# crstnbr/detqmc

Measured on AMD Instinct MI355X. Metric: DQMC sweeps/sec (SDW-O2 L=16 beta=10 fp64), higher is better.
Workload: dtype f64; 1 GPU; DetSDW O(2) L=16 beta=10 dtau=0.1 s=10 checkerboard delayed(32) sweepThermalization, 512 independent chains per GPU (1 process x 4 kernel contexts x 128 lockstep chains), stabilisation=qr; n_g=512, m=100, replicas_per_gpu=512, processes_per_gpu=1, contexts_per_process=4, chains_per_context=128, launch=self

## Files before the change

detqmc_amd/csrc/kernels_bmult.hip:

```cpp
#include "dqmc_internal.h"
#include <algorithm>
#include <cstdlib>
#include <mutex>

__device__ __forceinline__ cplx cadd(cplx a, cplx b) { return make_double2(a.x + b.x, a.y + b.y); }
__device__ __forceinline__ cplx cmul(cplx a, cplx b) {
    return make_double2(a.x * b.x - a.y * b.y, a.x * b.y + a.y * b.x);
}
__device__ __forceinline__ cplx cfma(cplx a, cplx b, cplx c) {
    c.x = fma(a.x, b.x, c.x); c.x = fma(-a.y, b.y, c.x);
    c.y = fma(a.x, b.y, c.y); c.y = fma(a.y, b.x, c.y);
    return c;
}
__device__ __forceinline__ cplx cscale(cplx a, double s) { return make_double2(a.x * s, a.y * s); }

template<int MSF>
__device__ __forceinline__ void build_V(cplx (&V)[MSF][MSF], double sign, double c0, double c1, double xs,
                                        double p0, double p1, double p2) {
#pragma unroll
    for (int a = 0; a < MSF; ++a)
#pragma unroll
        for (int b = 0; b < MSF; ++b) V[a][b] = make_double2(0.0, 0.0);
    cplx bx = make_double2(sign * p0 * xs, -sign * p1 * xs);
    cplx bcx = make_double2(sign * p0 * xs, sign * p1 * xs);
    V[0][0] = make_double2(c0, 0.0);
    V[1][1] = make_double2(c1, 0.0);
    V[0][1] = bx;
    V[1][0] = bcx;
    if (MSF == 4) {
        double ax = sign * p2 * xs;
        V[2][2] = make_double2(c0, 0.0);
        V[3][3] = make_double2(c1, 0.0);
        V[0][3] = make_double2(ax, 0.0);
        V[3][0] = make_double2(ax, 0.0);
        V[1][2] = make_double2(-ax, 0.0);
        V[2][1] = make_double2(-ax, 0.0);
        V[3][2] = bx;
        V[2][3] = bcx;
    }
}

template<int MSF, bool RIGHT, bool INV, bool CDW>
__global__ __launch_bounds__(512, MSF == 2 ? 4 : 2) void k_bmult_chain(DevModel dm, cplx* __restrict__ A, int lda, int nvec,
                                                      int kfirst, int kstep, int kcount, int shift, size_t cs) {
    extern __shared__ cplx sm[];
    dm = chain_model(dm, cs); CHAIN(A);
    const int N = dm.N, ng = dm.ng, P = dm.P;
    const int v0 = blockIdx.x * nvec;
    const int nv = min(nvec, ng - v0);
    if (nv <= 0) return;
    const int tid = threadIdx.x, nth = blockDim.x;
    const int rstride = nvec + 1;
    auto addr = [&](int v, int e) -> int { return RIGHT ? (e * rstride + v) : (v * ng + e); };

    const int rv0 = tid % nvec, re0 = tid / nvec, rvd = nth % nvec, red = nth / nvec;
    constexpr int SB = 8;
    if (!RIGHT) {
        const int total = nv * ng;
        const cplx* src = A + (size_t)v0 * lda;
        for (int base = tid; base < total; base += SB * nth) {
            cplx r[SB];
#pragma unroll
            for (int u = 0; u < SB; ++u) {
                const int idx = min(base + u * nth, total - 1);
                size_t off = idx;
                if (lda != ng) { const int v = idx / ng; off = (size_t)v * lda + (idx - v * ng); }
                r[u] = nt_load(src + off);
            }
#pragma unroll
            for (int u = 0; u < SB; ++u) { const int idx = base + u * nth; if (idx < total) sm[idx] = r[u]; }
        }
    } else {
        int v = rv0, e = re0;
        const int total = nvec * ng;
        for (int base = tid; base < total; base += SB * nth) {
            cplx r[SB];
            int la[SB];
#pragma unroll
            for (int u = 0; u < SB; ++u) {
                la[u] = (base + u * nth < total && v < nv) ? e * rstride + v : -1;
                r[u] = nt_load(A + (size_t)min(e, ng - 1) * lda + (v0 + min(v, nv - 1)));
                v += rvd; e += red;
                if (v >= nvec) { v -= nvec; e += 1; }
            }
#pragma unroll
            for (int u = 0; u < SB; ++u) if (la[u] >= 0) sm[la[u]] = r[u];
        }
    }
    __syncthreads();

    constexpr bool PASSES_FIRST = (RIGHT == INV);
    const int signIdx = INV ? 1 : 0;
    const double vsign = INV ? +1.0 : -1.0;

    int pl0[3], pld[3];
    if (!RIGHT) { pl0[0] = tid % P; pl0[1] = tid / P; pl0[2] = 0; pld[0] = nth % P; pld[1] = nth / P; pld[2] = 0; }
    else {
        pl0[0] = tid % nv; const int t0 = tid / nv; pl0[1] = t0 % P; pl0[2] = t0 / P;
        pld[0] = nth % nv; const int t1 = nth / nv; pld[1] = t1 % P; pld[2] = t1 / P;
    }
    const int si0 = tid % N, sv0 = tid / N, sid = nth % N, svd = nth / N;

    for (int kc = 0; kc < kcount; ++kc) {
        const int k = kfirst + kc * kstep;
        for (int stage = 0; stage < 2; ++stage) {
            const bool do_passes = (stage == 0) == PASSES_FIRST;
            if (shift && !do_passes) continue;
            if (do_passes) {
                if (dm.dense) continue;
                const double* abcd_tab = shift ? dm.pabcd_h : dm.pabcd;
                const cplx* mat_tab = shift ? dm.pmats_h : dm.pmats;
                const int npass = shift ? 2 : 3;
                for (int pass = 0; pass < npass; ++pass) {
                    const int sub = shift ? (pass == 0 ? 1 : 0) : ((pass == 1) ? 0 : 1);
                    if (!shift && pass == (PASSES_FIRST ? npass - 1 : 0)) {
                        const int fitems = nv * P;
                        const double* ph = dm.phi + (size_t)k * dm.opdim * N;
                        for (int idx = tid; idx < fitems; idx += nth) {
                            int p, v;
                            if (RIGHT) { v = idx % nv; p = idx / nv; } else { p = idx % P; v = idx / P; }
                            int site[4];
#pragma unroll
                            for (int q = 0; q < 4; ++q) site[q] = dm.psites[(sub * 4 + q) * P + p];
                            cplx x[MSF][4];
#pragma unroll
                            for (int b = 0; b < MSF; ++b)
#pragma unroll
                                for (int q = 0; q < 4; ++q) x[b][q] = sm[addr(v, b * N + site[q])];
                            auto vmix = [&]() {
#pragma unroll
                                for (int q = 0; q < 4; ++q) {
                                    const int i = site[q];
                                    const double c = dm.coshT[(size_t)k * N + i];
                                    double xs = dm.sinhT[(size_t)k * N + i], c0, c1;
                                    if constexpr (CDW) cdw_site_terms(dm, (size_t)k * N + i, vsign, c, c0, c1, xs); else { c0 = c; c1 = c; }
                                    const double p0 = ph[i];
                                    const double p1 = dm.opdim > 1 ? ph[N + i] : 0.0;
                                    const double p2 = dm.opdim > 2 ? ph[2 * N + i] : 0.0;
                                    cplx V[MSF][MSF];
                                    build_V<MSF>(V, vsign, c0, c1, xs, p0, p1, p2);
                                    cplx in[MSF], out[MSF];
#pragma unroll
                                    for (int b = 0; b < MSF; ++b) in[b] = x[b][q];
                                    if (PASSES_FIRST) {
#pragma unroll
                                        for (int b = 0; b < MSF; ++b) in[b] = cscale(in[b], INV ? dm.ovinv[b & 1] : dm.ov[b & 1]);
                                    }
#pragma unroll
                                    for (int o = 0; o < MSF; ++o) {
                                        cplx acc = make_double2(0.0, 0.0);
#pragma unroll
                                        for (int b = 0; b < MSF; ++b) {
                                            const cplx vv = RIGHT ? V[b][o] : V[o][b];
                                            acc = cfma(vv, in[b], acc);
                                        }
                                        if (!PASSES_FIRST) acc = cscale(acc, INV ? dm.ovinv[o & 1] : dm.ov[o & 1]);
                                        out[o] = acc;
                                    }
#pragma unroll
                                    for (int b = 0; b < MSF; ++b) x[b][q] = out[b];
                                }
                            };
                            if (!PASSES_FIRST) vmix();
#pragma unroll
                            for (int b = 0; b < MSF; ++b) {
                                const int tbl = ((b & 1) * 2 + signIdx) * 2 + sub;
                                cplx y[4];
                                if (dm.pm_real) {
                                    double co[4];
#pragma unroll
                                    for (int q = 0; q < 4; ++q) co[q] = abcd_tab[(tbl * 4 + q) * P + p];
#pragma unroll
                                    for (int a = 0; a < 4; ++a) {
                                        cplx acc = make_double2(0.0, 0.0);
#pragma unroll
                                        for (int q = 0; q < 4; ++q) {
                                            const double m = co[a ^ q];
                                            acc.x = fma(m, x[b][q].x, acc.x);
                                            acc.y = fma(m, x[b][q].y, acc.y);
                                        }
                                        y[a] = acc;
                                    }
                                } else {
                                    const cplx* mat = mat_tab + (size_t)tbl * 16 * P + p;
#pragma unroll
                                    for (int a = 0; a < 4; ++a) {
                                        cplx acc = make_double2(0.0, 0.0);
#pragma unroll
                                        for (int q = 0; q < 4; ++q) {
                                            const cplx mm = RIGHT ? mat[(size_t)(q * 4 + a) * P] : mat[(size_t)(a * 4 + q) * P];
                                            acc = cfma(mm, x[b][q], acc);
                                        }
                                        y[a] = acc;
                                    }
                                }
#pragma unroll
                                for (int q = 0; q < 4; ++q) x[b][q] = y[q];
                            }
                            if (PASSES_FIRST) vmix();
#pragma unroll
                            for (int b = 0; b < MSF; ++b)
#pragma unroll
                                for (int q = 0; q < 4; ++q) sm[addr(v, b * N + site[q])] = x[b][q];
                        }
                        __syncthreads();
                        continue;
                    }
                    const int items = nv * MSF * P;
                    int d0 = pl0[0], d1 = pl0[1], d2 = pl0[2];
                    for (int idx = tid; idx < items; idx += nth) {
                        int p, b, v;
                        if (RIGHT) { v = d0; p = d1; b = d2; }
                        else { p = d0; b = d1 % MSF; v = d1 / MSF; }
                        d0 += pld[0]; d1 += pld[1]; d2 += pld[2];
                        if (RIGHT) { if (d0 >= nv) { d0 -= nv; d1 += 1; } if (d1 >= P) { d1 -= P; d2 += 1; } }
                        else { if (d0 >= P) { d0 -= P; d1 += 1; } }
                        int band = b & 1;
                        const int tbl = (band * 2 + signIdx) * 2 + sub;
                        int e[4];
                        cplx x[4], y[4];
#pragma unroll
                        for (int q = 0; q < 4; ++q) { e[q] = addr(v, b * N + dm.psites[(sub * 4 + q) * P + p]); x[q] = sm[e[q]]; }
                        if (dm.pm_real) {
                            double co[4];
#pragma unroll
                            for (int q = 0; q < 4; ++q) co[q] = abcd_tab[(tbl * 4 + q) * P + p];
#pragma unroll
                            for (int a = 0; a < 4; ++a) {
                                cplx acc = make_double2(0.0, 0.0);
#pragma unroll
                                for (int q = 0; q < 4; ++q) {
                                    const double m = co[a ^ q];
                                    acc.x = fma(m, x[q].x, acc.x);
                                    acc.y = fma(m, x[q].y, acc.y);
                                }
                                y[a] = acc;
                            }
                        } else {
                            const cplx* mat = mat_tab + (size_t)tbl * 16 * P + p;
#pragma unroll
                            for (int a = 0; a < 4; ++a) {
                                cplx acc = make_double2(0.0, 0.0);
#pragma unroll
                                for (int q = 0; q < 4; ++q) {
                                    cplx mm = RIGHT ? mat[(size_t)(q * 4 + a) * P] : mat[(size_t)(a * 4 + q) * P];
                                    acc = cfma(mm, x[q], acc);
                                }
                                y[a] = acc;
                            }
                        }
#pragma unroll
                        for (int q = 0; q < 4; ++q) sm[e[q]] = y[q];
                    }
                    __syncthreads();
                }
            } else {
                if (!dm.dense) continue;
                const int items = nv * N;
                const double* ph = dm.phi + (size_t)k * dm.opdim * N;
                int i = si0, v = sv0, inext, vnext;
                for (int idx = tid; idx < items; idx += nth, i = inext, v = vnext) {
                    inext = i + sid; vnext = v + svd;
                    if (inext >= N) { inext -= N; vnext += 1; }
                    double c = dm.coshT[(size_t)k * N + i], xs = dm.sinhT[(size_t)k * N + i], c0, c1;
                    if constexpr (CDW) cdw_site_terms(dm, (size_t)k * N + i, vsign, c, c0, c1, xs); else { c0 = c; c1 = c; }
                    double p0 = ph[i];
                    double p1 = dm.opdim > 1 ? ph[N + i] : 0.0;
                    double p2 = dm.opdim > 2 ? ph[2 * N + i] : 0.0;
                    cplx V[MSF][MSF];
                    build_V<MSF>(V, vsign, c0, c1, xs, p0, p1, p2);
                    cplx in[MSF], out[MSF];
#pragma unroll
                    for (int q = 0; q < MSF; ++q) in[q] = sm[addr(v, q * N + i)];
                    if (PASSES_FIRST) {
#pragma unroll
                        for (int q = 0; q < MSF; ++q) in[q] = cscale(in[q], INV ? dm.ovinv[q & 1] : dm.ov[q & 1]);
                    }
#pragma unroll
                    for (int o = 0; o < MSF; ++o) {
                        cplx acc = make_double2(0.0, 0.0);
#pragma unroll
                        for (int q = 0; q < MSF; ++q) {
                            cplx vv = RIGHT ? V[q][o] : V[o][q];
                            acc = cfma(vv, in[q], acc);
                        }
                        if (!PASSES_FIRST) acc = cscale(acc, INV ? dm.ovinv[o & 1] : dm.ov[o & 1]);
                        out[o] = acc;
                    }
#pragma unroll
                    for (int q = 0; q < MSF; ++q) sm[addr(v, q * N + i)] = out[q];
                }
                __syncthreads();
            }
        }
    }

    if (!RIGHT) {
        cplx* dst = A + (size_t)v0 * lda;
        for (int idx = tid; idx < nv * ng; idx += nth) {
            size_t off = idx;
            if (lda != ng) { const int v = idx / ng; off = (size_t)v * lda + (idx - v * ng); }
            nt_store(dst + off, sm[idx]);
        }
    } else {
        int v = rv0, e = re0;
        for (int idx = tid; idx < nvec * ng; idx += nth) {
            if (v < nv) nt_store(A + (size_t)e * lda + (v0 + v), sm[e * rstride + v]);
            v += rvd; e += red;
            if (v >= nvec) { v -= nvec; e += 1; }
        }
    }
}

void launch_bmult(const Launch& lc, const DevModel* , const DevModel& hm, int side, int inverse,
                  int kfirst, int kstep, int kcount, cplx* A, int lda, int shift) {
    const int ng = hm.ng;
    const size_t lds_cap = side == DQMC_LEFT ? 65536 : 144 * 1024;
    const int max_fit = (int)(lds_cap / ((size_t)ng * sizeof(cplx))) - (side == DQMC_LEFT ? 0 : 1);
    static const int env_l = dev_knob("DQMC_BMULT_NVEC_L") ? atoi(dev_knob("DQMC_BMULT_NVEC_L")) : 0;
    static const int env_r = dev_knob("DQMC_BMULT_NVEC_R") ? atoi(dev_knob("DQMC_BMULT_NVEC_R")) : 0;
    int nvec;
    if (side == DQMC_LEFT) {
        const int per_pass = (256 + hm.P - 1) / hm.P;
        nvec = env_l ? env_l : std::max(ng / 256, per_pass);
        if (nvec > ng) nvec = ng;
    } else {
        nvec = env_r ? env_r : 8;
    }
    if (nvec > max_fit) nvec = max_fit;
    if (nvec < 1) nvec = 1;
    const int grid = (ng + nvec - 1) / nvec;
    const size_t lds = (size_t)(side == DQMC_LEFT ? nvec : nvec + 1) * ng * sizeof(cplx);
    if (lds > 48 * 1024) {
        static std::mutex mu;
        static size_t raised_tab[64][16] = {};
        int dev = 0;
        (void)hipGetDevice(&dev);
        const int slot = (hm.cdw_on ? 8 : 0) + (hm.MSF == 4 ? 4 : 0) + (side == DQMC_LEFT ? 0 : 2) + (inverse ? 1 : 0);
        std::lock_guard<std::mutex> lk(mu);
        size_t& raised = raised_tab[dev & 63][slot];
        if (lds > raised) {
            const void* f = nullptr;
#define BM_F(MSFV, R, I) (hm.cdw_on ? (const void*)k_bmult_chain<MSFV, R, I, true> : (const void*)k_bmult_chain<MSFV, R, I, false>)
            if (hm.MSF == 2) f = side == DQMC_LEFT ? (inverse ? BM_F(2, false, true) : BM_F(2, false, false)) : (inverse ? BM_F(2, true, true) : BM_F(2, true, false));
            else             f = side == DQMC_LEFT ? (inverse ? BM_F(4, false, true) : BM_F(4, false, false)) : (inverse ? BM_F(4, true, true) : BM_F(4, true, false));
#undef BM_F
            if (hipFuncSetAttribute(f, hipFuncAttributeMaxDynamicSharedMemorySize, (int)lds) == hipSuccess) raised = lds;
            else (void)hipGetLastError();
        }
    }
    static const int env_t = dev_knob("DQMC_BMULT_THREADS_R") ? atoi(dev_knob("DQMC_BMULT_THREADS_R")) : 0;
    const int nthreads = (side == DQMC_LEFT) ? 256 : (env_t ? env_t : (nvec >= 8 ? 512 : 256));
#define LAUNCH(MSFV, R, I)                                                                              \
    do { if (hm.cdw_on) hipLaunchKernelGGL((k_bmult_chain<MSFV, R, I, true>), dim3(grid, 1, lc.nb), dim3(nthreads), lds, lc.st, hm, A, lda, nvec, \
                                           kfirst, kstep, kcount, shift, lc.cs);                        \
         else hipLaunchKernelGGL((k_bmult_chain<MSFV, R, I, false>), dim3(grid, 1, lc.nb), dim3(nthreads), lds, lc.st, hm, A, lda, nvec, \
                                 kfirst, kstep, kcount, shift, lc.cs); } while (0)
    if (hm.MSF == 2) {
        if (side == DQMC_LEFT) { if (!inverse) LAUNCH(2, false, false); else LAUNCH(2, false, true); }
        else                   { if (!inverse) LAUNCH(2, true, false);  else LAUNCH(2, true, true); }
    } else {
        if (side == DQMC_LEFT) { if (!inverse) LAUNCH(4, false, false); else LAUNCH(4, false, true); }
        else                   { if (!inverse) LAUNCH(4, true, false);  else LAUNCH(4, true, true); }
    }
#undef LAUNCH
}

__global__ void k_cosh_sinh(DevModel dm, size_t cs) {
    dm = chain_model(dm, cs);
    const int total = dm.m * dm.N;
    for (int idx = blockIdx.x * blockDim.x + threadIdx.x; idx < total; idx += gridDim.x * blockDim.x) {
        int k = 1 + idx / dm.N, i = idx % dm.N;
        double nn = 0.0;
        for (int d = 0; d < dm.opdim; ++d) {
            double p = dm.phi[((size_t)k * dm.opdim + d) * dm.N + i];
            nn += p * p;
        }
        double nrm = sqrt(nn);
        double a = dm.lambda * dm.dtau * nrm;
        dm.coshT[(size_t)k * dm.N + i] = cosh(a);
        dm.sinhT[(size_t)k * dm.N + i] = sinh(a) / nrm;
    }
}
void launch_cosh_sinh(const Launch& lc, const DevModel& hm) {
    int total = hm.m * hm.N;
    hipLaunchKernelGGL(k_cosh_sinh, dim3((total + 255) / 256, 1, lc.nb), dim3(256), 0, lc.st, hm, lc.cs);
}

__global__ void k_cdw_terms(DevModel dm, size_t cs) {
    dm = chain_model(dm, cs);
    const int total = dm.m * dm.N;
    for (int idx = blockIdx.x * blockDim.x + threadIdx.x; idx < total; idx += gridDim.x * blockDim.x) {
        const size_t e = (size_t)dm.N + idx;
        const double l = dm.cdwl[e];
        const int a = (fabs(l) > 1.5) ? 1 : 0;
        dm.cdwC[e] = dm.cdw_cosh[a];
        dm.cdwS[e] = (l < 0.0) ? -dm.cdw_sinh[a] : dm.cdw_sinh[a];
    }
}
void launch_cdw_terms(const Launch& lc, const DevModel& hm) {
    if (!hm.cdw_on) return;
    int total = hm.m * hm.N;
    hipLaunchKernelGGL(k_cdw_terms, dim3((total + 255) / 256, 1, lc.nb), dim3(256), 0, lc.st, hm, lc.cs);
}

__global__ void k_set_identity(cplx* A, int n, size_t cs) {
    CHAIN(A);
    size_t total = (size_t)n * n;
    for (size_t idx = blockIdx.x * (size_t)blockDim.x + threadIdx.x; idx < total; idx += (size_t)gridDim.x * blockDim.x) {
        int i = (int)(idx % n), j = (int)(idx / n);
        A[idx] = make_double2(i == j ? 1.0 : 0.0, 0.0);
    }
}
void launch_set_identity(const Launch& lc, cplx* A, int n) {
    const int blocks = (int)std::min<size_t>(1024, ((size_t)n * n + 255) / 256);
    hipLaunchKernelGGL(k_set_identity, dim3(blocks, 1, lc.nb), dim3(256), 0, lc.st, A, n, lc.cs);
}

__global__ void k_conj_transpose(const cplx* __restrict__ A, cplx* __restrict__ B, int n, size_t cs) {
    __shared__ cplx tile[32][33];
    CHAIN(A); CHAIN(B);
    int bx = blockIdx.x * 32, by = blockIdx.y * 32;
    int tx = threadIdx.x & 31, ty = threadIdx.x >> 5;
    for (int r = ty; r < 32; r += 8) {
        int i = bx + tx, j = by + r;
        if (i < n && j < n) tile[r][tx] = A[(size_t)j * n + i];
    }
    __syncthreads();
    for (int r = ty; r < 32; r += 8) {
        int i = by + tx, j = bx + r;
        if (i < n && j < n) {
            cplx t = tile[tx][r];
            B[(size_t)j * n + i] = make_double2(t.x, -t.y);
        }
    }
}
void launch_conj_transpose(const Launch& lc, const cplx* A, cplx* B, int n) {
    dim3 grid((n + 31) / 32, (n + 31) / 32, lc.nb);
    hipLaunchKernelGGL(k_conj_transpose, grid, dim3(256), 0, lc.st, A, B, n, lc.cs);
}

__global__ void k_add_diag(cplx* A, const double* d, int n, size_t cs) {
    CHAIN(A); CHAIN(d);
    int i = blockIdx.x * blockDim.x + threadIdx.x;
    if (i < n) A[(size_t)i * n + i].x += d[i];
}
void launch_add_diag(const Launch& lc, cplx* A, const double* d, int n) {
    hipLaunchKernelGGL(k_add_diag, dim3((n + 255) / 256, 1, lc.nb), dim3(256), 0, lc.st, A, d, n, lc.cs);
}

__global__ void k_copy64(const unsigned long long* __restrict__ src, unsigned long long* __restrict__ dst, size_t words, size_t cs) {
    CHAIN(src); CHAIN(dst);
    for (size_t i = blockIdx.x * (size_t)blockDim.x + threadIdx.x; i < words; i += (size_t)gridDim.x * blockDim.x) dst[i] = src[i];
}
void launch_copy_bytes(const Launch& lc, const void* src, void* dst, size_t bytes) {
    if (lc.nb == 1) { (void)hipMemcpyAsync(dst, src, bytes, hipMemcpyDeviceToDevice, lc.st); return; }
    const size_t words = bytes / 8;
    const int blocks = (int)std::min<size_t>(2048, (words + 255) / 256);
    hipLaunchKernelGGL(k_copy64, dim3(blocks, 1, lc.nb), dim3(256), 0, lc.st, (const unsigned long long*)src,
                       (unsigned long long*)dst, words, lc.cs);
}
void launch_copy(const Launch& lc, const cplx* A, cplx* B, size_t count) {
    launch_copy_bytes(lc, A, B, count * sizeof(cplx));
}

__global__ void k_phi_sq_sum(DevModel dm, double* out, size_t cs) {
    __shared__ double red[256];
    dm = chain_model(dm, cs); CHAIN(out);
    double acc = 0.0;
    size_t total = (size_t)dm.m * dm.opdim * dm.N;
    const double* p = dm.phi + (size_t)dm.opdim * dm.N;
    for (size_t idx = threadIdx.x; idx < total; idx += 256) acc += p[idx] * p[idx];
    red[threadIdx.x] = acc;
    __syncthreads();
    for (int s = 128; s > 0; s >>= 1) {
        if ((int)threadIdx.x < s) red[threadIdx.x] += red[threadIdx.x + s];
        __syncthreads();
    }
    if (threadIdx.x == 0) out[0] = red[0];
}
__global__ void k_phi_action(DevModel dm, const DevUpdateState* __restrict__ us, double* out, size_t cs) {
    __shared__ double red[256];
    dm = chain_model(dm, cs); CHAIN(us); CHAIN(out);
    const int N = dm.N, L = dm.L, m = dm.m, OPD = dm.opdim;
    const double dtau = dm.dtau, r = us->r, u = dm.u, c = dm.c;
    double acc = 0.0;
    for (int idx = threadIdx.x; idx < m * N; idx += 256) {
        const int k = 1 + idx / N, site = idx % N;
        const int kprev = (k > 1) ? k - 1 : m;
        const int x = site % L, y = site / L;
        const int xn = y * L + (x + 1) % L, yn = ((y + 1) % L) * L + x;
        double phisq = 0.0, td2 = 0.0, xd2 = 0.0, yd2 = 0.0;
        for (int d = 0; d < OPD; ++d) {
            const double ph = dm.phi[((size_t)k * OPD + d) * N + site];
            const double td = (ph - dm.phi[((size_t)kprev * OPD + d) * N + site]) / dtau;
            const double xd = ph - dm.phi[((size_t)k * OPD + d) * N + xn];
            const double yd = ph - dm.phi[((size_t)k * OPD + d) * N + yn];
            td2 += td * td; xd2 += xd * xd; yd2 += yd * yd; phisq += ph * ph;
        }
        double a = 0.5 * dtau * r * phisq;
        if (!dm.phi2bosons) a += (dtau / (2.0 * c * c)) * td2 + 0.5 * dtau * xd2 + 0.5 * dtau * yd2 + 0.25 * dtau * u * phisq * phisq;
        acc += a;
    }
    red[threadIdx.x] = acc;
    __syncthreads();
    for (int s = 128; s > 0; s >>= 1) {
        if ((int)threadIdx.x < s) red[threadIdx.x] += red[threadIdx.x + s];
        __syncthreads();
    }
    if (threadIdx.x == 0) out[0] = red[0];
}
void launch_phi_action(const Launch& lc, const DevModel& hm, const DevUpdateState* us, double* out) {
    hipLaunchKernelGGL(k_phi_action, dim3(1, 1, lc.nb), dim3(256), 0, lc.st, hm, us, out, lc.cs);
}
__global__ void k_phi_shift(DevModel dm, const double* __restrict__ shifts, size_t cs) {
    dm = chain_model(dm, cs);
    const double* sh = shifts + (size_t)blockIdx.z * dm.opdim;
    const int total = (dm.m + 1) * dm.opdim * dm.N;
    for (int idx = blockIdx.x * blockDim.x + threadIdx.x; idx < total; idx += gridDim.x * blockDim.x)
        dm.phi[idx] += sh[(idx / dm.N) % dm.opdim];
}
void launch_phi_shift(const Launch& lc, const DevModel& hm, const double* shifts) {
    const int total = (hm.m + 1) * hm.opdim * hm.N;
    hipLaunchKernelGGL(k_phi_shift, dim3((total + 255) / 256, 1, lc.nb), dim3(256), 0, lc.st, hm, shifts, lc.cs);
}
void launch_phi_sq_sum(const Launch& lc, const DevModel& hm, double* out) {
    hipLaunchKernelGGL(k_phi_sq_sum, dim3(1, 1, lc.nb), dim3(256), 0, lc.st, hm, out, lc.cs);
}
__global__ void k_gather_scalars(const double* __restrict__ src, size_t cs, int nb, double factor, double* __restrict__ dst) {
    const int b = blockIdx.x * blockDim.x + threadIdx.x;
    if (b < nb) dst[b] = factor * *(const double*)((const char*)src + (size_t)b * cs);
}
void launch_gather_scalars(const Launch& lc, const double* src, double factor, double* dst) {
    hipLaunchKernelGGL(k_gather_scalars, dim3((lc.nb + 63) / 64), dim3(64), 0, lc.st, src, lc.cs, lc.nb, factor, dst);
}
```

Baseline: 283.8 sweeps/s.

## Fuse checkerboard passes across time slices and stream edges from global memory

Restructures the chained B-matrix multiply so the outer sub-lattice pass of one time slice is merged with the matching pass of the next slice, with the potential mixing step folded in. This removes one pass and one barrier per interior slice. Optionally the first pass reads directly from global memory and the last pass writes directly back, skipping the bulk shared-memory load and store. Defaults enable all three for right multiplies and only the mid fusion for left; this relies on the pass-1 sub-lattice operators composing, and the direct global accesses are scattered rather than coalesced.

```diff
diff --git a/detqmc_amd/csrc/kernels_bmult.hip b/detqmc_amd/csrc/kernels_bmult.hip
--- a/detqmc_amd/csrc/kernels_bmult.hip
+++ b/detqmc_amd/csrc/kernels_bmult.hip
@@ -42,7 +42,7 @@
 
 template<int MSF, bool RIGHT, bool INV, bool CDW>
 __global__ __launch_bounds__(512, MSF == 2 ? 4 : 2) void k_bmult_chain(DevModel dm, cplx* __restrict__ A, int lda, int nvec,
-                                                      int kfirst, int kstep, int kcount, int shift, size_t cs) {
+                                                      int kfirst, int kstep, int kcount, int shift, int fuse, size_t cs) {
     extern __shared__ cplx sm[];
     dm = chain_model(dm, cs); CHAIN(A);
     const int N = dm.N, ng = dm.ng, P = dm.P;
@@ -52,249 +52,274 @@
     const int tid = threadIdx.x, nth = blockDim.x;
     const int rstride = nvec + 1;
     auto addr = [&](int v, int e) -> int { return RIGHT ? (e * rstride + v) : (v * ng + e); };
+    auto gaddr = [&](int v, int e) -> size_t { return RIGHT ? ((size_t)e * lda + (v0 + v)) : ((size_t)(v0 + v) * lda + e); };
+
+    const bool fuse_in = !dm.dense && (fuse & 1);
+    const bool fuse_out = !dm.dense && !shift && (fuse & 2);
+    const bool fuse_mid = (fuse & 4) != 0;
 
     const int rv0 = tid % nvec, re0 = tid / nvec, rvd = nth % nvec, red = nth / nvec;
-    constexpr int SB = 8;
-    if (!RIGHT) {
-        const int total = nv * ng;
-        const cplx* src = A + (size_t)v0 * lda;
-        for (int base = tid; base < total; base += SB * nth) {
-            cplx r[SB];
-#pragma unroll
-            for (int u = 0; u < SB; ++u) {
-                const int idx = min(base + u * nth, total - 1);
-                size_t off = idx;
-                if (lda != ng) { const int v = idx / ng; off = (size_t)v * lda + (idx - v * ng); }
-                r[u] = nt_load(src + off);
+    if (!fuse_in) {
+        constexpr int SB = 8;
+        if (!RIGHT) {
+            const int total = nv * ng;
+            const cplx* src = A + (size_t)v0 * lda;
+            for (int base = tid; base < total; base += SB * nth) {
+                cplx r[SB];
+#pragma unroll
+                for (int u = 0; u < SB; ++u) {
+                    const int idx = min(base + u * nth, total - 1);
+                    size_t off = idx;
+                    if (lda != ng) { const int v = idx / ng; off = (size_t)v * lda + (idx - v * ng); }
+                    r[u] = nt_load(src + off);
+                }
+#pragma unroll
+                for (int u = 0; u < SB; ++u) { const int idx = base + u * nth; if (idx < total) sm[idx] = r[u]; }
             }
-#pragma unroll
-            for (int u = 0; u < SB; ++u) { const int idx = base + u * nth; if (idx < total) sm[idx] = r[u]; }
-        }
-    } else {
-        int v = rv0, e = re0;
-        const int total = nvec * ng;
-        for (int base = tid; base < total; base += SB * nth) {
-            cplx r[SB];
-            int la[SB];
-#pragma unroll
-            for (int u = 0; u < SB; ++u) {
-                la[u] = (base + u * nth < total && v < nv) ? e * rstride + v : -1;
-                r[u] = nt_load(A + (size_t)min(e, ng - 1) * lda + (v0 + min(v, nv - 1)));
-                v += rvd; e += red;
-                if (v >= nvec) { v -= nvec; e += 1; }
+        } else {
+            int v = rv0, e = re0;
+            const int total = nvec * ng;
+            for (int base = tid; base < total; base += SB * nth) {
+                cplx r[SB];
+                int la[SB];
+#pragma unroll
+                for (int u = 0; u < SB; ++u) {
+                    la[u] = (base + u * nth < total && v < nv) ? e * rstride + v : -1;
+                    r[u] = nt_load(A + (size_t)min(e, ng - 1) * lda + (v0 + min(v, nv - 1)));
+                    v += rvd; e += red;
+                    if (v >= nvec) { v -= nvec; e += 1; }
+                }
+#pragma unroll
+                for (int u = 0; u < SB; ++u) if (la[u] >= 0) sm[la[u]] = r[u];
             }
-#pragma unroll
-            for (int u = 0; u < SB; ++u) if (la[u] >= 0) sm[la[u]] = r[u];
-        }
-    }
-    __syncthreads();
+        }
+        __syncthreads();
+    }
 
     constexpr bool PASSES_FIRST = (RIGHT == INV);
     const int signIdx = INV ? 1 : 0;
     const double vsign = INV ? +1.0 : -1.0;
 
-    int pl0[3], pld[3];
-    if (!RIGHT) { pl0[0] = tid % P; pl0[1] = tid / P; pl0[2] = 0; pld[0] = nth % P; pld[1] = nth / P; pld[2] = 0; }
-    else {
-        pl0[0] = tid % nv; const int t0 = tid / nv; pl0[1] = t0 % P; pl0[2] = t0 / P;
-        pld[0] = nth % nv; const int t1 = nth / nv; pld[1] = t1 % P; pld[2] = t1 / P;
-    }
-    const int si0 = tid % N, sv0 = tid / N, sid = nth % N, svd = nth / N;
-
-    for (int kc = 0; kc < kcount; ++kc) {
-        const int k = kfirst + kc * kstep;
-        for (int stage = 0; stage < 2; ++stage) {
-            const bool do_passes = (stage == 0) == PASSES_FIRST;
-            if (shift && !do_passes) continue;
-            if (do_passes) {
-                if (dm.dense) continue;
-                const double* abcd_tab = shift ? dm.pabcd_h : dm.pabcd;
-                const cplx* mat_tab = shift ? dm.pmats_h : dm.pmats;
-                const int npass = shift ? 2 : 3;
-                for (int pass = 0; pass < npass; ++pass) {
-                    const int sub = shift ? (pass == 0 ? 1 : 0) : ((pass == 1) ? 0 : 1);
-                    if (!shift && pass == (PASSES_FIRST ? npass - 1 : 0)) {
-                        const int fitems = nv * P;
-                        const double* ph = dm.phi + (size_t)k * dm.opdim * N;
-                        for (int idx = tid; idx < fitems; idx += nth) {
-                            int p, v;
-                            if (RIGHT) { v = idx % nv; p = idx / nv; } else { p = idx % P; v = idx / P; }
-                            int site[4];
-#pragma unroll
-                            for (int q = 0; q < 4; ++q) site[q] = dm.psites[(sub * 4 + q) * P + p];
-                            cplx x[MSF][4];
-#pragma unroll
-                            for (int b = 0; b < MSF; ++b)
-#pragma unroll
-                                for (int q = 0; q < 4; ++q) x[b][q] = sm[addr(v, b * N + site[q])];
-                            auto vmix = [&]() {
-#pragma unroll
-                                for (int q = 0; q < 4; ++q) {
-                                    const int i = site[q];
-                                    const double c = dm.coshT[(size_t)k * N + i];
-                                    double xs = dm.sinhT[(size_t)k * N + i], c0, c1;
-                                    if constexpr (CDW) cdw_site_terms(dm, (size_t)k * N + i, vsign, c, c0, c1, xs); else { c0 = c; c1 = c; }
-                                    const double p0 = ph[i];
-                                    const double p1 = dm.opdim > 1 ? ph[N + i] : 0.0;
-                                    const double p2 = dm.opdim > 2 ? ph[2 * N + i] : 0.0;
-                                    cplx V[MSF][MSF];
-                                    build_V<MSF>(V, vsign, c0, c1, xs, p0, p1, p2);
-                                    cplx in[MSF], out[MSF];
-#pragma unroll
-                                    for (int b = 0; b < MSF; ++b) in[b] = x[b][q];
-                                    if (PASSES_FIRST) {
-#pragma unroll
-                                        for (int b = 0; b < MSF; ++b) in[b] = cscale(in[b], INV ? dm.ovinv[b & 1] : dm.ov[b & 1]);
+    if (!dm.dense) {
+        const double* abcd_tab = shift ? dm.pabcd_h : dm.pabcd;
+        const cplx* mat_tab = shift ? dm.pmats_h : dm.pmats;
+        int pl0[3], pld[3];
+        if (!RIGHT) { pl0[0] = tid % P; pl0[1] = tid / P; pl0[2] = 0; pld[0] = nth % P; pld[1] = nth / P; pld[2] = 0; }
+        else {
+            pl0[0] = tid % nv; const int t0 = tid / nv; pl0[1] = t0 % P; pl0[2] = t0 / P;
+            pld[0] = nth % nv; const int t1 = nth / nv; pld[1] = t1 % P; pld[2] = t1 / P;
+        }
+        const int nj = shift ? kcount : kcount + 1;
+        for (int j = 0; j < nj; ++j) {
+            const int nparts = (!fuse_mid && !shift && j > 0 && j < kcount) ? 2 : 1;
+            for (int part = 0; part < nparts; ++part) {
+                const bool h_a = !shift && j > 0 && (nparts == 1 || part == 0);
+                const bool h_b = (shift || j < kcount) && (nparts == 1 || part == 1);
+                int kv = -1;
+                if (!shift) {
+                    if (PASSES_FIRST) { if (j > 0 && part == 0) kv = kfirst + (j - 1) * kstep; }
+                    else if (j < kcount && part == nparts - 1) kv = kfirst + j * kstep;
+                }
+                const bool from_g = fuse_in && j == 0, to_g = fuse_out && j == kcount;
+                const int fitems = nv * P;
+                for (int idx = tid; idx < fitems; idx += nth) {
+                    int p, v;
+                    if (RIGHT) { v = idx % nv; p = idx / nv; } else { p = idx % P; v = idx / P; }
+                    int site[4];
+#pragma unroll
+                    for (int q = 0; q < 4; ++q) site[q] = dm.psites[(4 + q) * P + p];
+                    cplx x[MSF][4];
+                    if (from_g) {
+#pragma unroll
+                        for (int b = 0; b < MSF; ++b)
+#pragma unroll
+                            for (int q = 0; q < 4; ++q) x[b][q] = nt_load(A + gaddr(v, b * N + site[q]));
+                    } else {
+#pragma unroll
+                        for (int b = 0; b < MSF; ++b)
+#pragma unroll
+                            for (int q = 0; q < 4; ++q) x[b][q] = sm[addr(v, b * N + site[q])];
+                    }
+                    auto hstep = [&]() {
+#pragma unroll
+                        for (int b = 0; b < MSF; ++b) {
+                            cplx y[4];
+                            if (dm.pm_real) {
+                                double co[4];
+#pragma unroll
+                                for (int q = 0; q < 4; ++q) co[q] = abcd_tab[((((b & 1) * 2 + signIdx) * 2 + 1) * 4 + q) * P + p];
+#pragma unroll
+                                for (int a = 0; a < 4; ++a) {
+                                    cplx acc = make_double2(0.0, 0.0);
+#pragma unroll
+                                    for (int q = 0; q < 4; ++q) {
+                                        const double m = co[a ^ q];
+                                        acc.x = fma(m, x[b][q].x, acc.x);
+                                        acc.y = fma(m, x[b][q].y, acc.y);
                                     }
-#pragma unroll
-                                    for (int o = 0; o < MSF; ++o) {
-                                        cplx acc = make_double2(0.0, 0.0);
-#pragma unroll
-                                        for (int b = 0; b < MSF; ++b) {
-                                            const cplx vv = RIGHT ? V[b][o] : V[o][b];
-                                            acc = cfma(vv, in[b], acc);
-                                        }
-                                        if (!PASSES_FIRST) acc = cscale(acc, INV ? dm.ovinv[o & 1] : dm.ov[o & 1]);
-                                        out[o] = acc;
+                                    y[a] = acc;
+                                }
+                            } else {
+                                const int tbl = ((b & 1) * 2 + signIdx) * 2 + 1;
+                                const cplx* mat = mat_tab + (size_t)tbl * 16 * P + p;
+#pragma unroll
+                                for (int a = 0; a < 4; ++a) {
+                                    cplx acc = make_double2(0.0, 0.0);
+#pragma unroll
+                                    for (int q = 0; q < 4; ++q) {
+                                        const cplx mm = RIGHT ? mat[(size_t)(q * 4 + a) * P] : mat[(size_t)(a * 4 + q) * P];
+                                        acc = cfma(mm, x[b][q], acc);
                                     }
-#pragma unroll
-                                    for (int b = 0; b < MSF; ++b) x[b][q] = out[b];
+                                    y[a] = acc;
                                 }
-                            };
-                            if (!PASSES_FIRST) vmix();
-#pragma unroll
-                            for (int b = 0; b < MSF; ++b) {
-                                const int tbl = ((b & 1) * 2 + signIdx) * 2 + sub;
-                                cplx y[4];
-                                if (dm.pm_real) {
-                                    double co[4];
-#pragma unroll
-                                    for (int q = 0; q < 4; ++q) co[q] = abcd_tab[(tbl * 4 + q) * P + p];
-#pragma unroll
-                                    for (int a = 0; a < 4; ++a) {
-                                        cplx acc = make_double2(0.0, 0.0);
-#pragma unroll
-                                        for (int q = 0; q < 4; ++q) {
-                                            const double m = co[a ^ q];
-                                            acc.x = fma(m, x[b][q].x, acc.x);
-                                            acc.y = fma(m, x[b][q].y, acc.y);
-                                        }
-                                        y[a] = acc;
-                                    }
-                                } else {
-                                    const cplx* mat = mat_tab + (size_t)tbl * 16 * P + p;
-#pragma unroll
-                                    for (int a = 0; a < 4; ++a) {
-                                        cplx acc = make_double2(0.0, 0.0);
-#pragma unroll
-                                        for (int q = 0; q < 4; ++q) {
-                                            const cplx mm = RIGHT ? mat[(size_t)(q * 4 + a) * P] : mat[(size_t)(a * 4 + q) * P];
-                                            acc = cfma(mm, x[b][q], acc);
-                                        }
-                                        y[a] = acc;
-                                    }
+                            }
+#pragma unroll
+                            for (int q = 0; q < 4; ++q) x[b][q] = y[q];
+                        }
+                    };
+                    if (h_a) hstep();
+                    if (kv >= 0) {
+                        const double* ph = dm.phi + (size_t)kv * dm.opdim * N;
+#pragma unroll
+                        for (int q = 0; q < 4; ++q) {
+                            const int i = site[q];
+                            const double c = dm.coshT[(size_t)kv * N + i];
+                            double xs = dm.sinhT[(size_t)kv * N + i], c0, c1;
+                            if constexpr (CDW) cdw_site_terms(dm, (size_t)kv * N + i, vsign, c, c0, c1, xs); else { c0 = c; c1 = c; }
+                            const double p0 = ph[i];
+                            const double p1 = dm.opdim > 1 ? ph[N + i] : 0.0;
+                            const double p2 = dm.opdim > 2 ? ph[2 * N + i] : 0.0;
+                            cplx V[MSF][MSF];
+                            build_V<MSF>(V, vsign, c0, c1, xs, p0, p1, p2);
+                            cplx in[MSF], out[MSF];
+#pragma unroll
+                            for (int b = 0; b < MSF; ++b) in[b] = x[b][q];
+                            if (PASSES_FIRST) {
+#pragma unroll
+                                for (int b = 0; b < MSF; ++b) in[b] = cscale(in[b], INV ? dm.ovinv[b & 1] : dm.ov[b & 1]);
+                            }
+#pragma unroll
+                            for (int o = 0; o < MSF; ++o) {
+                                cplx acc = make_double2(0.0, 0.0);
+#pragma unroll
+                                for (int b = 0; b < MSF; ++b) {
+                                    const cplx vv = RIGHT ? V[b][o] : V[o][b];
+                                    acc = cfma(vv, in[b], acc);
                                 }
-#pragma unroll
-                                for (int q = 0; q < 4; ++q) x[b][q] = y[q];
+                                if (!PASSES_FIRST) acc = cscale(acc, INV ? dm.ovinv[o & 1] : dm.ov[o & 1]);
+                                out[o] = acc;
                             }
-                            if (PASSES_FIRST) vmix();
-#pragma unroll
-                            for (int b = 0; b < MSF; ++b)
-#pragma unroll
-                                for (int q = 0; q < 4; ++q) sm[addr(v, b * N + site[q])] = x[b][q];
+#pragma unroll
+                            for (int b = 0; b < MSF; ++b) x[b][q] = out[b];
                         }
-                        __syncthreads();
-                        continue;
                     }
-                    const int items = nv * MSF * P;
-                    int d0 = pl0[0], d1 = pl0[1], d2 = pl0[2];
-                    for (int idx = tid; idx < items; idx += nth) {
-                        int p, b, v;
-                        if (RIGHT) { v = d0; p = d1; b = d2; }
-                        else { p = d0; b = d1 % MSF; v = d1 / MSF; }
-                        d0 += pld[0]; d1 += pld[1]; d2 += pld[2];
-                        if (RIGHT) { if (d0 >= nv) { d0 -= nv; d1 += 1; } if (d1 >= P) { d1 -= P; d2 += 1; } }
-                        else { if (d0 >= P) { d0 -= P; d1 += 1; } }
-                        int band = b & 1;
-                        const int tbl = (band * 2 + signIdx) * 2 + sub;
-                        int e[4];
-                        cplx x[4], y[4];
-#pragma unroll
-                        for (int q = 0; q < 4; ++q) { e[q] = addr(v, b * N + dm.psites[(sub * 4 + q) * P + p]); x[q] = sm[e[q]]; }
-                        if (dm.pm_real) {
-                            double co[4];
-#pragma unroll
-                            for (int q = 0; q < 4; ++q) co[q] = abcd_tab[(tbl * 4 + q) * P + p];
-#pragma unroll
-                            for (int a = 0; a < 4; ++a) {
-                                cplx acc = make_double2(0.0, 0.0);
-#pragma unroll
-                                for (int q = 0; q < 4; ++q) {
-                                    const double m = co[a ^ q];
-                                    acc.x = fma(m, x[q].x, acc.x);
-                                    acc.y = fma(m, x[q].y, acc.y);
-                                }
-                                y[a] = acc;
-                            }
-                        } else {
-                            const cplx* mat = mat_tab + (size_t)tbl * 16 * P + p;
-#pragma unroll
-                            for (int a = 0; a < 4; ++a) {
-                                cplx acc = make_double2(0.0, 0.0);
-#pragma unroll
-                                for (int q = 0; q < 4; ++q) {
-                                    cplx mm = RIGHT ? mat[(size_t)(q * 4 + a) * P] : mat[(size_t)(a * 4 + q) * P];
-                                    acc = cfma(mm, x[q], acc);
-                                }
-                                y[a] = acc;
-                            }
+                    if (h_b) hstep();
+                    if (to_g) {
+#pragma unroll
+                        for (int b = 0; b < MSF; ++b)
+#pragma unroll
+                            for (int q = 0; q < 4; ++q) nt_store(A + gaddr(v, b * N + site[q]), x[b][q]);
+                    } else {
+#pragma unroll
+                        for (int b = 0; b < MSF; ++b)
+#pragma unroll
+                            for (int q = 0; q < 4; ++q) sm[addr(v, b * N + site[q])] = x[b][q];
+                    }
+                }
+                if (!to_g) __syncthreads();
+            }
+            if (!shift && j == kcount) break;
+            const int items = nv * MSF * P;
+            int d0 = pl0[0], d1 = pl0[1], d2 = pl0[2];
+            for (int idx = tid; idx < items; idx += nth) {
+                int p, b, v;
+                if (RIGHT) { v = d0; p = d1; b = d2; }
+                else { p = d0; b = d1 % MSF; v = d1 / MSF; }
+                d0 += pld[0]; d1 += pld[1]; d2 += pld[2];
+                if (RIGHT) { if (d0 >= nv) { d0 -= nv; d1 += 1; } if (d1 >= P) { d1 -= P; d2 += 1; } }
+                else { if (d0 >= P) { d0 -= P; d1 += 1; } }
+                int band = b & 1;
+                const int tbl = (band * 2 + signIdx) * 2;
+                int e[4];
+                cplx x[4], y[4];
+#pragma unroll
+                for (int q = 0; q < 4; ++q) { e[q] = addr(v, b * N + dm.psites[q * P + p]); x[q] = sm[e[q]]; }
+                if (dm.pm_real) {
+                    double co[4];
+#pragma unroll
+                    for (int q = 0; q < 4; ++q) co[q] = abcd_tab[(tbl * 4 + q) * P + p];
+#pragma unroll
+                    for (int a = 0; a < 4; ++a) {
+                        cplx acc = make_double2(0.0, 0.0);
+#pragma unroll
+                        for (int q = 0; q < 4; ++q) {
+                            const double m = co[a ^ q];
+                            acc.x = fma(m, x[q].x, acc.x);
+                            acc.y = fma(m, x[q].y, acc.y);
                         }
-#pragma unroll
-                        for (int q = 0; q < 4; ++q) sm[e[q]] = y[q];
+                        y[a] = acc;
                     }
-                    __syncthreads();
-                }
-            } else {
-                if (!dm.dense) continue;
-                const int items = nv * N;
-                const double* ph = dm.phi + (size_t)k * dm.opdim * N;
-                int i = si0, v = sv0, inext, vnext;
-                for (int idx = tid; idx < items; idx += nth, i = inext, v = vnext) {
-                    inext = i + sid; vnext = v + svd;
-                    if (inext >= N) { inext -= N; vnext += 1; }
-                    double c = dm.coshT[(size_t)k * N + i], xs = dm.sinhT[(size_t)k * N + i], c0, c1;
-                    if constexpr (CDW) cdw_site_terms(dm, (size_t)k * N + i, vsign, c, c0, c1, xs); else { c0 = c; c1 = c; }
-                    double p0 = ph[i];
-                    double p1 = dm.opdim > 1 ? ph[N + i] : 0.0;
-                    double p2 = dm.opdim > 2 ? ph[2 * N + i] : 0.0;
-                    cplx V[MSF][MSF];
-                    build_V<MSF>(V, vsign, c0, c1, xs, p0, p1, p2);
-                    cplx in[MSF], out[MSF];
-#pragma unroll
-                    for (int q = 0; q < MSF; ++q) in[q] = sm[addr(v, q * N + i)];
-                    if (PASSES_FIRST) {
-#pragma unroll
-                        for (int q = 0; q < MSF; ++q) in[q] = cscale(in[q], INV ? dm.ovinv[q & 1] : dm.ov[q & 1]);
+                } else {
+                    const cplx* mat = mat_tab + (size_t)tbl * 16 * P + p;
+#pragma unroll
+                    for (int a = 0; a < 4; ++a) {
+                        cplx acc = make_double2(0.0, 0.0);
+#pragma unroll
+                        for (int q = 0; q < 4; ++q) {
+                            cplx mm = RIGHT ? mat[(size_t)(q * 4 + a) * P] : mat[(size_t)(a * 4 + q) * P];
+                            acc = cfma(mm, x[q], acc);
+                        }
+                        y[a] = acc;
                     }
-#pragma unroll
-                    for (int o = 0; o < MSF; ++o) {
-                        cplx acc = make_double2(0.0, 0.0);
-#pragma unroll
-                        for (int q = 0; q < MSF; ++q) {
-                            cplx vv = RIGHT ? V[q][o] : V[o][q];
-                            acc = cfma(vv, in[q], acc);
-                        }
-                        if (!PASSES_FIRST) acc = cscale(acc, INV ? dm.ovinv[o & 1] : dm.ov[o & 1]);
-                        out[o] = acc;
+                }
+#pragma unroll
+                for (int q = 0; q < 4; ++q) sm[e[q]] = y[q];
+            }
+            __syncthreads();
+        }
+    } else if (!shift) {
+        const int si0 = tid % N, sv0 = tid / N, sid = nth % N, svd = nth / N;
+        for (int kc = 0; kc < kcount; ++kc) {
+            const int k = kfirst + kc * kstep;
+            const int items = nv * N;
+            const double* ph = dm.phi + (size_t)k * dm.opdim * N;
+            int i = si0, v = sv0, inext, vnext;
+            for (int idx = tid; idx < items; idx += nth, i = inext, v = vnext) {
+                inext = i + sid; vnext = v + svd;
+                if (inext >= N) { inext -= N; vnext += 1; }
+                double c = dm.coshT[(size_t)k * N + i], xs = dm.sinhT[(size_t)k * N + i], c0, c1;
+                if constexpr (CDW) cdw_site_terms(dm, (size_t)k * N + i, vsign, c, c0, c1, xs); else { c0 = c; c1 = c; }
+                double p0 = ph[i];
+                double p1 = dm.opdim > 1 ? ph[N + i] : 0.0;
+                double p2 = dm.opdim > 2 ? ph[2 * N + i] : 0.0;
+                cplx V[MSF][MSF];
+                build_V<MSF>(V, vsign, c0, c1, xs, p0, p1, p2);
+                cplx in[MSF], out[MSF];
+#pragma unroll
+                for (int q = 0; q < MSF; ++q) in[q] = sm[addr(v, q * N + i)];
+                if (PASSES_FIRST) {
+#pragma unroll
+                    for (int q = 0; q < MSF; ++q) in[q] = cscale(in[q], INV ? dm.ovinv[q & 1] : dm.ov[q & 1]);
+                }
+#pragma unroll
+                for (int o = 0; o < MSF; ++o) {
+                    cplx acc = make_double2(0.0, 0.0);
+#pragma unroll
+                    for (int q = 0; q < MSF; ++q) {
+                        cplx vv = RIGHT ? V[q][o] : V[o][q];
+                        acc = cfma(vv, in[q], acc);
                     }
-#pragma unroll
-                    for (int q = 0; q < MSF; ++q) sm[addr(v, q * N + i)] = out[q];
-                }
-                __syncthreads();
+                    if (!PASSES_FIRST) acc = cscale(acc, INV ? dm.ovinv[o & 1] : dm.ov[o & 1]);
+                    out[o] = acc;
+                }
+#pragma unroll
+                for (int q = 0; q < MSF; ++q) sm[addr(v, q * N + i)] = out[q];
             }
-        }
-    }
-
+            __syncthreads();
+        }
+    }
+
+    if (fuse_out) return;
     if (!RIGHT) {
         cplx* dst = A + (size_t)v0 * lda;
         for (int idx = tid; idx < nv * ng; idx += nth) {
@@ -319,6 +344,8 @@
     const int max_fit = (int)(lds_cap / ((size_t)ng * sizeof(cplx))) - (side == DQMC_LEFT ? 0 : 1);
     static const int env_l = dev_knob("DQMC_BMULT_NVEC_L") ? atoi(dev_knob("DQMC_BMULT_NVEC_L")) : 0;
     static const int env_r = dev_knob("DQMC_BMULT_NVEC_R") ? atoi(dev_knob("DQMC_BMULT_NVEC_R")) : 0;
+    static const int env_f = dev_knob("DQMC_BMULT_FUSE") ? atoi(dev_knob("DQMC_BMULT_FUSE")) & 7 : -1;
+    const int fuse = env_f >= 0 ? env_f : (side == DQMC_LEFT ? 4 : 7);
     int nvec;
     if (side == DQMC_LEFT) {
         const int per_pass = (256 + hm.P - 1) / hm.P;
@@ -353,9 +380,9 @@
     const int nthreads = (side == DQMC_LEFT) ? 256 : (env_t ? env_t : (nvec >= 8 ? 512 : 256));
 #define LAUNCH(MSFV, R, I)                                                                              \
     do { if (hm.cdw_on) hipLaunchKernelGGL((k_bmult_chain<MSFV, R, I, true>), dim3(grid, 1, lc.nb), dim3(nthreads), lds, lc.st, hm, A, lda, nvec, \
-                                           kfirst, kstep, kcount, shift, lc.cs);                        \
+                                           kfirst, kstep, kcount, shift, fuse, lc.cs);                        \
          else hipLaunchKernelGGL((k_bmult_chain<MSFV, R, I, false>), dim3(grid, 1, lc.nb), dim3(nthreads), lds, lc.st, hm, A, lda, nvec, \
-                                 kfirst, kstep, kcount, shift, lc.cs); } while (0)
+                                 kfirst, kstep, kcount, shift, fuse, lc.cs); } while (0)
     if (hm.MSF == 2) {
         if (side == DQMC_LEFT) { if (!inverse) LAUNCH(2, false, false); else LAUNCH(2, false, true); }
         else                   { if (!inverse) LAUNCH(2, true, false);  else LAUNCH(2, true, true); }
```

Result: no change. 285.4 sweeps/s, median of 6 (+0.6%).
